# pierrenodet/spark-ensemble

Hardware: AMD Instinct MI355X
Metric: rows/sec (whole node) GBMClassifier 100 trees depth=8 at 1/2/4/8 MI355X (higher is better)
Workload: dtype fp32; 1 GPU; model=GBMClassifier(bernoulli, 265 trees, depth=8, bins=256), global_batch=10000000, rows_per_gpu=10000000, features=256, parallelism=dp1

## Files before the change

csrc/hist_plan.h:

```cpp
#pragma once

#include <algorithm>
#include <cmath>
#include <cstddef>
#include <cstdint>
#include <cstdlib>
#include <limits>
#include <stdexcept>
#include <vector>

struct HistPlan {
  int64_t chunk_rows = 0;
  int n_chunks = 0;
  int header_words = 0;
  std::vector<int> table;
  std::vector<int> multi_nodes;
};

inline HistPlan plan_hist_chunks(const int64_t* offs, int n_nodes,
                                 const int* col0 ,
                                 int64_t row_bound, int col_bound,
                                 size_t lds_bytes, int n_groups,
                                 int header_words) {
  int64_t total_rows = 0;
  for (int nd = 0; nd < n_nodes; ++nd) {
    const int64_t s = offs[nd], e = offs[nd + 1];
    if (s < 0 || e < s || e > row_bound ||
        e > std::numeric_limits<int>::max())
      throw std::invalid_argument("hist plan: node_offsets out of range");
    const int c0 = col0 ? col0[nd] : 0;
    if (c0 < 0 || c0 >= col_bound)
      throw std::invalid_argument("hist plan: node_col0 out of range");
    total_rows += e - s;
  }

  const int blocks_per_cu =
      std::max<int>(1, (int)(163840 / std::max<size_t>(1, lds_bytes)));
  const int64_t resident = (int64_t)256 * blocks_per_cu;
  static const double oversub_env = []() {
    const char* e = getenv("SEA_HIST_OVERSUB");
    return e ? atof(e) : 0.0;
  }();
  const double oversub =
      oversub_env > 0 ? oversub_env : (blocks_per_cu == 1 ? 1.0 : 1.5);
  const int64_t target_chunks = std::max<int64_t>(
      1, (int64_t)(resident * oversub) / std::max(1, n_groups));

  HistPlan p;
  p.chunk_rows = std::max<int64_t>(
      4096, (total_rows + target_chunks - 1) / target_chunks);
  p.chunk_rows = std::min<int64_t>(p.chunk_rows, 1 << 20);
  p.header_words = header_words;
  p.table.assign(header_words, 0);
  for (int nd = 0; nd < n_nodes; ++nd) {
    const int64_t s = offs[nd], e = offs[nd + 1];
    int slot = -1;
    if (e - s > p.chunk_rows) {
      slot = (int)p.multi_nodes.size();
      p.multi_nodes.push_back(nd);
    }
    int64_t c = s;
    do {
      const int rec[5] = {nd, (int)c,
                          (int)std::min<int64_t>(p.chunk_rows, e - c), slot,
                          col0 ? col0[nd] : 0};
      p.table.insert(p.table.end(), rec, rec + 5);
      c += p.chunk_rows;
    } while (c < e);
  }
  p.n_chunks = (int)((p.table.size() - header_words) / 5);
  return p;
}

inline double hist_fixed_scale(int64_t chunk_rows, double max_abs) {
  if (!(max_abs > 0.0) || !std::isfinite(max_abs)) max_abs = 1.0;
  const double s = (double)(1u << 30) / ((double)chunk_rows * max_abs);
  return std::min(s, (double)(1u << 30) / max_abs);
}
```

csrc/ops.hip:

```cpp

#include <ATen/hip/HIPContext.h>

#include <chrono>
#include <cstring>
#include <tuple>
#include <vector>

#include "common.h"
#include "hist_plan.h"

torch::Tensor h2d_async(const void* src, size_t bytes, UploadSlot slot,
                        const torch::Device& dev) {
  static thread_local torch::Tensor pin[2 * kUploadSlots];
  static thread_local hipEvent_t done[2 * kUploadSlots] = {};
  static thread_local unsigned char flip[kUploadSlots] = {};
  flip[slot] ^= 1;
  const int bi = slot * 2 + flip[slot];
  auto& b = pin[bi];
  if (done[bi]) (void)hipEventSynchronize(done[bi]);
  if (!b.defined() || (size_t)b.numel() < bytes) {
    size_t cap = 4096;
    while (cap < bytes) cap *= 2;
    b = torch::empty({(int64_t)cap},
                     torch::TensorOptions().dtype(torch::kByte)
// ... 98 lines not shown
      while (lo < hi) {
        const int mid = (lo + hi) >> 1;
        if (e[mid] >= v[j]) hi = mid; else lo = mid + 1;
      }
      b[j] = (uint8_t)lo;
    }
    if (full) {
      uint4 packed;
      unsigned* w = reinterpret_cast<unsigned*>(&packed);
#pragma unroll
      for (int q = 0; q < 4; ++q)
        w[q] = (unsigned)b[q * 4] | ((unsigned)b[q * 4 + 1] << 8) |
               ((unsigned)b[q * 4 + 2] << 16) | ((unsigned)b[q * 4 + 3] << 24);
      *reinterpret_cast<uint4*>(out + r * F + f0) = packed;
    } else {
      for (int j = 0; j < nf; ++j) out[r * F + f0 + j] = b[j];
    }
  }
}

void bin_features(torch::Tensor out, torch::Tensor x, torch::Tensor edges) {
  CHECK_GPU(out); CHECK_GPU(x); CHECK_GPU(edges);
  CHECK_CONTIG(out); CHECK_CONTIG(x); CHECK_CONTIG(edges);
  int64_t n = x.size(0);
  int F = (int)x.size(1);
  int nedges = (int)edges.size(1);
  TORCH_CHECK(nedges <= 1024, "bin_features: too many edges for LDS staging");
  auto stream = at::hip::getCurrentHIPStream();
  const int threads = 256;
  const int fgroups = (int)ceil_div(F, 16);
  int rblocks = (int)std::min<int64_t>(
      ceil_div(n, threads), std::max<int64_t>(1, 16384 / fgroups));
  const size_t lds = (size_t)16 * nedges * 4;
  hipLaunchKernelGGL(bin_features_kernel, dim3(rblocks, fgroups),
                     dim3(threads), lds, stream, out.data_ptr<uint8_t>(),
                     x.data_ptr<float>(), edges.data_ptr<float>(), n, F,
                     nedges);
}


__device__ inline void rotate_piece(unsigned (&w)[4], int lam) {
  const bool r1 = lam & 4, r2 = lam & 8;
  const unsigned a0 = r1 ? w[1] : w[0], a1 = r1 ? w[2] : w[1],
                 a2 = r1 ? w[3] : w[2], a3 = r1 ? w[0] : w[3];
  const unsigned b0 = r2 ? a2 : a0, b1 = r2 ? a3 : a1, b2 = r2 ? a0 : a2,
                 b3 = r2 ? a1 : a3;
  const unsigned t = lam & 3;
  w[0] = __builtin_amdgcn_alignbyte(b1, b0, t);
  w[1] = __builtin_amdgcn_alignbyte(b2, b1, t);
  w[2] = __builtin_amdgcn_alignbyte(b3, b2, t);
  w[3] = __builtin_amdgcn_alignbyte(b0, b3, t);
}

template <int DC, int NC, bool BM>
__global__ void hist_build_kernel(
    float* __restrict__ out,
    long long* __restrict__ stage,
    const uint8_t* __restrict__ bins,
    const float* __restrict__ gh,
    const int* __restrict__ row_idx,
    const int* __restrict__ chunks,
    int F, int B, int FG, int CH, int identity_rows) {
  constexpr int C = DC + NC;
  constexpr int CELLS = DC > NC ? DC : NC;
  extern __shared__ unsigned long long lds64[];
  const float* scales = reinterpret_cast<const float*>(chunks);
  const int* chk = chunks + 2 * C + blockIdx.x * 5;
  const int fg = blockIdx.y;
  const int f0 = fg * FG;
  const int nf = min(FG, F - f0);
  const int node = chk[0];
  const int start = chk[1];
  const int len = chk[2];
  const int slot = chk[3];
  const int col0 = chk[4];

  const int lds_cells = FG * B * CELLS;
  for (int i = threadIdx.x; i < lds_cells; i += blockDim.x) lds64[i] = 0ull;
  __syncthreads();

  constexpr int MAXNH = CELLS == 1 ? 4 : (CELLS == 2 ? 2 : 1);
  const int nh = FG >> 4;
  const int lam = threadIdx.x & 15;
  const int bshift = 31 - __clz(FG) + 3;
  const unsigned plane = (unsigned)B * FG * 8;
  unsigned foff[16];
#pragma unroll
  for (int p = 0; p < 16; ++p) foff[p] = ((p + lam) & 15) * 8;

  for (int i = threadIdx.x; i < len; i += blockDim.x) {
    const int r = identity_rows ? start + i : row_idx[start + i];
    const float* g = gh + (int64_t)r * CH + col0;
    unsigned long long addend[CELLS];
#pragma unroll
    for (int c = 0; c < CELLS; ++c) addend[c] = 0ull;
#pragma unroll
    for (int d = 0; d < DC; ++d) {
      const int iv = __float2int_rn(g[d] * scales[d]);
      addend[d] |= ((unsigned long long)(unsigned)iv) << 32;
    }
#pragma unroll
    for (int c = 0; c < NC; ++c) {
      const int iv = __float2int_rn(g[DC + c] * scales[DC + c]);
      addend[c] |= (unsigned)iv;
    }
    if constexpr (BM) {
      const uint8_t* br = bins + (int64_t)r * F + f0;
      uint4 bv[MAXNH];
#pragma unroll
      for (int hh = 0; hh < MAXNH; ++hh) {
        bv[hh] = make_uint4(0, 0, 0, 0);
        if (hh < nh) bv[hh] = *reinterpret_cast<const uint4*>(br + 16 * hh);
      }
      char* base = reinterpret_cast<char*>(lds64);
#pragma unroll
      for (int hh = 0; hh < MAXNH; ++hh) {
        if (hh >= nh) break;
        unsigned w[4] = {bv[hh].x, bv[hh].y, bv[hh].z, bv[hh].w};
        rotate_piece(w, lam);
#pragma unroll
        for (int p = 0; p < 16; ++p) {
          const unsigned b = (w[p >> 2] >> (8 * (p & 3))) & 0xff;
          char* cell = base + ((b << bshift) + foff[p]) + hh * 128;
#pragma unroll
          for (int c = 0; c < CELLS; ++c)
            atomicAdd(reinterpret_cast<unsigned long long*>(cell + c * plane),
                      addend[c]);
        }
      }
    } else {
      const uint8_t* br = bins + (int64_t)r * F + f0;
      for (int f = 0; f < nf; ++f) {
        const int b = br[f];
        unsigned long long* cell = lds64 + ((f * B) + b) * CELLS;
#pragma unroll
        for (int c = 0; c < CELLS; ++c) atomicAdd(cell + c, addend[c]);
      }
    }
  }
  __syncthreads();

  auto flush_cell = [&](int f, int b, const unsigned long long* cell,
                        int cstride) {
    if (slot < 0) {
      float* o = out + (((int64_t)node * F + f0 + f) * B + b) * C;
#pragma unroll
      for (int d = 0; d < DC; ++d)
        o[d] = (float)(int)(unsigned)(cell[d * cstride] >> 32) / scales[d];
#pragma unroll
      for (int c = 0; c < NC; ++c)
        o[DC + c] = (float)(int)(unsigned)(cell[c * cstride] & 0xFFFFFFFFull) /
                    scales[DC + c];
    } else {
      long long* o = stage + (((int64_t)slot * F + f0 + f) * B + b) * C;
#pragma unroll
      for (int d = 0; d < DC; ++d) {
        const int v = (int)(unsigned)(cell[d * cstride] >> 32);
        if (v) atomicAdd((unsigned long long*)(o + d),
                         (unsigned long long)(long long)v);
      }
#pragma unroll
      for (int c = 0; c < NC; ++c) {
        const int v = (int)(unsigned)(cell[c * cstride] & 0xFFFFFFFFull);
        if (v) atomicAdd((unsigned long long*)(o + DC + c),
                         (unsigned long long)(long long)v);
      }
    }
  };
  if constexpr (BM) {
    constexpr int TBL = 3;
    constexpr int TB = 1 << TBL, TF = 64 >> TBL;
    const int nbt = (B + TB - 1) >> TBL;
    const int n_tiles = (FG / TF) * nbt;
    for (int i = threadIdx.x; i < n_tiles * 64; i += blockDim.x) {
      const int t = i >> 6, l = i & 63;
      const int ft = t / nbt, bt = t - ft * nbt;
      const int f = ft * TF + (l >> TBL), b = bt * TB + (l & (TB - 1));
      if (b < B) flush_cell(f, b, lds64 + b * FG + f, B * FG);
    }
  } else {
    for (int i = threadIdx.x; i < nf * B; i += blockDim.x) {
      const int f = i / B, b = i - f * B;
      flush_cell(f, b, lds64 + ((f * B) + b) * CELLS, 1);
    }
  }
}

__global__ void hist_decode_kernel(float* __restrict__ out,
                                   const long long* __restrict__ stage,
                                   const int* __restrict__ nodes,
                                   const float* __restrict__ scales,
                                   int64_t FBC, int C) {
  const int64_t obase = (int64_t)nodes[blockIdx.y] * FBC;
  const int64_t sbase = (int64_t)blockIdx.y * FBC;
  for (int64_t i = blockIdx.x * (int64_t)blockDim.x + threadIdx.x; i < FBC;
       i += gridDim.x * (int64_t)blockDim.x) {
    const int c = (int)(i % C);
    out[obase + i] = (float)stage[sbase + i] / scales[c];
  }
}

void launch_hist_decode(float* out, const long long* stage, const int* nodes,
                        const float* scales, int n_multi, int64_t FBC, int C,
                        hipStream_t stream) {
  const int dblocks = (int)std::min<int64_t>(ceil_div(FBC, 256), 1024);
  hipLaunchKernelGGL(hist_decode_kernel, dim3(dblocks, n_multi), dim3(256), 0,
                     stream, out, stage, nodes, scales, FBC, C);
}

int64_t hist_build(torch::Tensor out, torch::Tensor bins, torch::Tensor gh,
                   torch::Tensor row_idx, torch::Tensor node_offsets,
                   int64_t num_bins, int64_t d_dims, torch::Tensor max_abs,
                   bool identity_rows, torch::Tensor node_col0,
                   int64_t c_per_node) {
  CHECK_GPU(out); CHECK_GPU(bins); CHECK_GPU(gh); CHECK_GPU(row_idx);
  CHECK_CONTIG(out); CHECK_CONTIG(bins); CHECK_CONTIG(gh); CHECK_CONTIG(row_idx);
  TORCH_CHECK(!node_offsets.is_cuda(), "node_offsets stays on host");
  TORCH_CHECK(!max_abs.is_cuda(), "max_abs stays on host");
  TORCH_CHECK(!node_col0.is_cuda(), "node_col0 stays on host");
  CHECK_CONTIG(node_offsets); CHECK_CONTIG(node_col0);
  const int F = (int)bins.size(1);
  const int B = (int)num_bins;
  const int CH = (int)gh.size(1);
  const int C = c_per_node > 0 ? (int)c_per_node : CH;
  const int n_nodes = (int)node_offsets.numel() - 1;
  const bool forest = node_col0.numel() > 0;
  TORCH_CHECK(!forest || node_col0.numel() == n_nodes,
              "node_col0 must have one entry per node");
  const int D = d_dims > 0 ? (int)d_dims : (C >= 3 ? C - 2 : C - 1);
  const int NN = C - D;
  TORCH_CHECK(C <= 8, "gh channels capped at 8 (grad dims + hess + count)");
  TORCH_CHECK(D >= 1 && NN >= 1 && NN <= 2,
              "hist_build: channels must be D grads + 1-2 nonneg, got C=", C,
              " D=", D);
  TORCH_CHECK(max_abs.numel() == C, "max_abs must have C entries");
  TORCH_CHECK(out.numel() == (int64_t)n_nodes * F * B * C,
              "out must be [n_nodes, F, B, C]");
  if (n_nodes == 0 || F == 0) return 0;
  const int CELLS = std::max(D, NN);

  static const int fg_env = []() {
    const char* e = getenv("SEA_HIST_FG");
    return e ? atoi(e) : 0;
  }();
  static const int lds_budget = []() {
    const char* e = getenv("SEA_HIST_LDS");
    return e ? atoi(e) : 163840;
  }();
  int FG = std::max<int>(1, std::min<int>(F, lds_budget / (B * CELLS * 8)));
  if (CELLS == 1 && FG >= 64 && (F % 64) == 0) FG = 64;
  else if (CELLS <= 2 && FG >= 32 && (F % 32) == 0) FG = 32;
  else if (FG >= 16) FG = 16;
  else if (FG >= 8) FG = 8;
  else if (FG >= 4) FG = 4;
  if (fg_env == 16 || fg_env == 32 || fg_env == 64)
    FG = std::min(FG, fg_env);
  const int threads =
      (FG >= 64 || (CELLS == 2 && FG >= 32)) ? 1024
      : ((FG >= 32 || (CELLS >= 3 && FG >= 16)) ? 512 : 256);
  const int n_groups = (int)ceil_div(F, FG);
  const size_t lds_bytes = (size_t)FG * B * CELLS * 8;

  HistPlan plan = plan_hist_chunks(
      node_offsets.data_ptr<int64_t>(), n_nodes,
      forest ? node_col0.data_ptr<int>() : nullptr,
      identity_rows ? bins.size(0) : row_idx.numel(), CH - C + 1, lds_bytes,
      n_groups, 2 * C);

  auto max_abs_f = max_abs.to(torch::kFloat32).contiguous();
  auto ma = max_abs_f.accessor<float, 1>();
  float* scales_f = reinterpret_cast<float*>(plan.table.data());
  for (int c = 0; c < C; ++c)
    scales_f[c] = (float)hist_fixed_scale(plan.chunk_rows, ma[c]);
  auto chunks = h2d_async(plan.table.data(), plan.table.size() * 4,
                          kSlotHistChunks, bins.device())
                    .view(torch::kInt32);

  const int n_multi = (int)plan.multi_nodes.size();
  torch::Tensor stage;
  long long* stage_ptr = nullptr;
  if (n_multi) {
    stage = torch::zeros({(int64_t)n_multi, (int64_t)F, (int64_t)B, (int64_t)C},
                         out.options().dtype(torch::kInt64));
    stage_ptr = reinterpret_cast<long long*>(stage.data_ptr<int64_t>());
  }

  auto stream = at::hip::getCurrentHIPStream();
  const bool bin_major =
      (FG == 16 || FG == 32 || FG == 64) && (F % FG) == 0;
  TORCH_CHECK(!bin_major || FG <= (CELLS == 1 ? 64 : (CELLS == 2 ? 32 : 16)),
              "hist_build: FG ", FG, " too wide for CELLS ", CELLS);
#define HB_LAUNCH_L(DD, NNN, BM)                                             \
  do {                                                                       \
    if (lds_bytes > 65536)                                                   \
      (void)hipFuncSetAttribute(                                             \
          reinterpret_cast<const void*>(&hist_build_kernel<DD, NNN, BM>),    \
          hipFuncAttributeMaxDynamicSharedMemorySize, (int)lds_bytes);       \
    hipLaunchKernelGGL((hist_build_kernel<DD, NNN, BM>),                     \
                       dim3(plan.n_chunks, n_groups), dim3(threads),         \
                       lds_bytes, stream, out.data_ptr<float>(), stage_ptr,  \
                       bins.data_ptr<uint8_t>(),                             \
                       gh.data_ptr<float>(), row_idx.data_ptr<int>(),        \
                       chunks.data_ptr<int>(), F, B, FG, CH,                 \
                       identity_rows ? 1 : 0);                               \
  } while (0)
#define HB_LAUNCH(DD, NNN)                                                   \
  do {                                                                       \
    if (bin_major) HB_LAUNCH_L(DD, NNN, true);                               \
    else HB_LAUNCH_L(DD, NNN, false);                                        \
  } while (0)
  const int key = D * 10 + NN;
  switch (key) {
    case 11: HB_LAUNCH(1, 1); break;
    case 12: HB_LAUNCH(1, 2); break;
    case 21: HB_LAUNCH(2, 1); break;
    case 22: HB_LAUNCH(2, 2); break;
    case 31: HB_LAUNCH(3, 1); break;
    case 32: HB_LAUNCH(3, 2); break;
    case 41: HB_LAUNCH(4, 1); break;
    case 42: HB_LAUNCH(4, 2); break;
    case 51: HB_LAUNCH(5, 1); break;
    case 52: HB_LAUNCH(5, 2); break;
    case 61: HB_LAUNCH(6, 1); break;
    case 62: HB_LAUNCH(6, 2); break;
    case 71: HB_LAUNCH(7, 1); break;
    default: TORCH_CHECK(false, "hist_build: unsupported D/NN ", D, "/", NN);
  }
#undef HB_LAUNCH
#undef HB_LAUNCH_L
  if (n_multi) {
    auto nodes = h2d_async(plan.multi_nodes.data(), (size_t)n_multi * 4,
                           kSlotHistNodes, bins.device());
    launch_hist_decode(out.data_ptr<float>(), stage_ptr,
                       (const int*)nodes.data_ptr(),
                       reinterpret_cast<const float*>(chunks.data_ptr<int>()),
                       n_multi, (int64_t)F * B * C, C, stream);
  }
  return n_multi;
}


__global__ void partition_kernel(
    int* __restrict__ new_rows,
    int* __restrict__ cursors,
    const uint8_t* __restrict__ bins,
    const uint8_t* __restrict__ bins_t,
    const int* __restrict__ row_idx,
    const int* __restrict__ chunks,
    const int* __restrict__ feat,
    const int* __restrict__ thr,
    int F, long long Nrows) {
  __shared__ int base_l, base_r, loc_l, loc_r;
  __shared__ int wl[8];
  extern __shared__ unsigned long long bits[];
  const int chunk = blockIdx.x;
  const int node = chunks[chunk * 3 + 0];
  const int start = chunks[chunk * 3 + 1];
  const int len = chunks[chunk * 3 + 2];
  const int f = feat[node];
  const int t = thr[node];
  const int lane = threadIdx.x & 63;
  const int wave = threadIdx.x >> 6;

  int my_l = 0;
  for (int i = threadIdx.x; i < ((len + 63) & ~63); i += blockDim.x) {
    const bool active = i < len;
    bool left = false;
    if (active) {
      const int r = row_idx[start + i];
      if (f < 0) {
        left = true;
      } else {
        const uint8_t bv = bins_t ? bins_t[(int64_t)f * Nrows + r]
                                  : bins[(int64_t)r * F + f];
        left = bv <= t;
      }
    }
    const unsigned long long m = __ballot(active && left);
    if (lane == 0) {
      bits[i >> 6] = m;
      my_l += (int)__popcll(m);
    }
  }
// ... 236 lines not shown
          const uint8_t bv = xt ? br[(int64_t)f * n] : br[f];
          go_left = bv <= (unsigned)(nd >> 32);
        } else {
          go_left = xr[f] <= __uint_as_float((unsigned)(nd >> 32));
        }
        node = toff + left + (go_left ? 0 : 1);
        nd = tlds[node];
        f = (short)(nd & 0xFFFFu);
      }
      if (D1) {
        acc1 += __uint_as_float((unsigned)(nd >> 32));
      } else {
        const float wt = w[first_tree + t];
        const float* lv = leaf + (int64_t)(node_base + node) * D;
        for (int d = 0; d < D; ++d) acc[d] += wt * lv[d];
      }
    }
    if (D1) {
      atomicAdd(out + r, acc1);
    } else {
      float* o = out + r * D;
      for (int d = 0; d < D; ++d)
        if (acc[d] != 0.0f) atomicAdd(o + d, acc[d]);
    }
  }
}


__device__ inline int seg_of(const long long* __restrict__ cum, int n_segs,
                             long long p) {
  int lo = 0, hi = n_segs;
  while (hi - lo > 1) {
    const int mid = (lo + hi) >> 1;
    if (cum[mid] <= p) lo = mid; else hi = mid;
  }
  return lo;
}

__global__ void gather_ranges_kernel(
    int* __restrict__ out,
    const int* __restrict__ src,
    const long long* __restrict__ seg,
    int n_segs, long long total) {
  const long long* cum = seg;
  const long long* starts = seg + n_segs + 1;
  const long long stride = (long long)gridDim.x * blockDim.x;
  for (long long p = (long long)blockIdx.x * blockDim.x + threadIdx.x;
       p < total; p += stride) {
    const int s = seg_of(cum, n_segs, p);
    out[p] = src[starts[s] + (p - cum[s])];
  }
}

__global__ void leaf_scatter_kernel(
    float* __restrict__ tp,
    const int* __restrict__ row_idx,
    const long long* __restrict__ seg,
    const int* __restrict__ tree,
    const float* __restrict__ val,
    int T, int n_segs, long long total) {
  const long long* cum = seg;
  const long long* starts = seg + n_segs + 1;
  const long long stride = (long long)gridDim.x * blockDim.x;
  for (long long p = (long long)blockIdx.x * blockDim.x + threadIdx.x;
       p < total; p += stride) {
    const int s = seg_of(cum, n_segs, p);
    const int r = row_idx[starts[s] + (p - cum[s])];
    tp[(long long)r * T + tree[s]] = val[s];
  }
}

void gather_ranges(torch::Tensor out, torch::Tensor src,
                   torch::Tensor starts, torch::Tensor lens) {
  CHECK_GPU(out); CHECK_GPU(src);
  const int n_segs = (int)starts.numel();
  const long long total = out.numel();
  if (n_segs == 0 || total == 0) return;
  auto st = starts.accessor<int64_t, 1>();
  auto ln = lens.accessor<int64_t, 1>();
  std::vector<long long> seg_v(2 * n_segs + 1);
  seg_v[0] = 0;
  for (int i = 0; i < n_segs; ++i) {
    seg_v[i + 1] = seg_v[i] + ln[i];
    seg_v[n_segs + 1 + i] = st[i];
  }
  TORCH_CHECK(seg_v[n_segs] == total, "gather_ranges: lens sum != out size");
  auto seg_b = h2d_async(seg_v.data(), seg_v.size() * 8, kSlotGatherSegs,
                         src.device());
  auto stream = at::hip::getCurrentHIPStream();
  const int blocks =
      (int)std::min<long long>(8192, ceil_div(total, (long long)1024));
  hipLaunchKernelGGL(gather_ranges_kernel, dim3(blocks), dim3(256), 0, stream,
                     out.data_ptr<int>(), src.data_ptr<int>(),
                     (const long long*)seg_b.data_ptr(), n_segs, total);
}

void leaf_scatter(torch::Tensor tp, torch::Tensor row_idx,
                  torch::Tensor starts, torch::Tensor lens,
                  torch::Tensor tree, torch::Tensor val) {
  CHECK_GPU(tp); CHECK_GPU(row_idx);
  const int n_segs = (int)starts.numel();
  if (n_segs == 0) return;
  const int T = (int)tp.size(1);
  auto st = starts.accessor<int64_t, 1>();
  auto ln = lens.accessor<int64_t, 1>();
  std::vector<long long> seg_v(2 * n_segs + 1);
  seg_v[0] = 0;
  for (int i = 0; i < n_segs; ++i) {
    seg_v[i + 1] = seg_v[i] + ln[i];
    seg_v[n_segs + 1 + i] = st[i];
  }
  const long long total = seg_v[n_segs];
  if (total == 0) return;
  auto seg_b = h2d_async(seg_v.data(), seg_v.size() * 8, kSlotLeafSegs,
                         tp.device());
  std::vector<int> tv(n_segs);
  std::vector<float> vv(n_segs);
  auto ta = tree.accessor<int64_t, 1>();
  auto va = val.accessor<float, 1>();
  for (int i = 0; i < n_segs; ++i) { tv[i] = (int)ta[i]; vv[i] = va[i]; }
  auto tree_b = h2d_async(tv.data(), tv.size() * 4, kSlotLeafTree, tp.device());
  std::vector<char> vb(n_segs * 4);
  std::memcpy(vb.data(), vv.data(), n_segs * 4);
  auto val_b = h2d_async(vb.data(), vb.size(), kSlotLeafVal, tp.device());
  auto stream = at::hip::getCurrentHIPStream();
  const int blocks =
      (int)std::min<long long>(8192, ceil_div(total, (long long)1024));
  hipLaunchKernelGGL(leaf_scatter_kernel, dim3(blocks), dim3(256), 0, stream,
                     tp.data_ptr<float>(), row_idx.data_ptr<int>(),
                     (const long long*)seg_b.data_ptr(),
                     (const int*)tree_b.data_ptr(),
                     (const float*)val_b.data_ptr(), T, n_segs, total);
}


__global__ void transpose_u8_kernel(uint8_t* __restrict__ out,
                                    const uint8_t* __restrict__ in,
                                    int64_t n, int F) {
  __shared__ uint8_t tile[64][68];
  const int64_t r0 = (int64_t)blockIdx.x * 64;
  const int f0 = blockIdx.y * 64;
  const int tid = threadIdx.x;
  const bool full = (r0 + 64 <= n) && (f0 + 64 <= F) && ((F & 3) == 0) &&
                    ((n & 3) == 0);
  if (full) {
    for (int i = tid; i < 1024; i += 256) {
      const int rr = i >> 4;
// ... 570 lines not shown
  if (C > 8) {
    CHECK_GPU(gain); CHECK_GPU(feat); CHECK_GPU(bin); CHECK_GPU(left_stats);
    split_argmax_wide(gain, feat, bin, left_stats, hist, D, lam,
                      min_child_weight, min_instances, min_info_gain);
    return;
  }
  auto best = torch::zeros({n}, hist.options().dtype(torch::kInt64));
  auto stream = at::hip::getCurrentHIPStream();
  const int fpb = 4;
#define SA_LAUNCH(CC)                                                         \
  do {                                                                        \
    hipLaunchKernelGGL(split_argmax_kernel<CC>,                               \
                       dim3(n, (F + fpb - 1) / fpb), dim3(64 * fpb), 0,       \
                       stream,                                                \
                       (unsigned long long*)best.data_ptr<int64_t>(),         \
                       hist.data_ptr<float>(), F, B, D, (float)lam,           \
                       (float)min_child_weight, (float)min_instances);        \
    hipLaunchKernelGGL(split_decode_kernel<CC>, dim3(n), dim3(64), 0, stream, \
                       gain.data_ptr<float>(), feat.data_ptr<int>(),          \
                       bin.data_ptr<int>(), left_stats.data_ptr<float>(),     \
                       (unsigned long long*)best.data_ptr<int64_t>(),         \
                       hist.data_ptr<float>(), F, B, (float)min_info_gain);   \
  } while (0)
  switch (C) {
    case 2: SA_LAUNCH(2); break;
    case 3: SA_LAUNCH(3); break;
    case 4: SA_LAUNCH(4); break;
    case 5: SA_LAUNCH(5); break;
    case 6: SA_LAUNCH(6); break;
    case 7: SA_LAUNCH(7); break;
    case 8: SA_LAUNCH(8); break;
  }
#undef SA_LAUNCH
}

std::tuple<int64_t, torch::Tensor, torch::Tensor> hist_plan_debug(
    torch::Tensor node_offsets, torch::Tensor node_col0, int64_t row_bound,
    int64_t col_bound, int64_t lds_bytes, int64_t n_groups) {
  auto offs = node_offsets.to(torch::kInt64).contiguous();
  auto col0 = node_col0.to(torch::kInt32).contiguous();
  const int n_nodes = (int)offs.numel() - 1;
  TORCH_CHECK(col0.numel() == 0 || col0.numel() == n_nodes,
              "node_col0 must be empty or have one entry per node");
  HistPlan plan = plan_hist_chunks(
      offs.data_ptr<int64_t>(), n_nodes,
      col0.numel() ? col0.data_ptr<int>() : nullptr, row_bound,
      (int)col_bound, (size_t)lds_bytes, (int)n_groups, 0);
  auto i32 = torch::TensorOptions().dtype(torch::kInt32);
  auto chunks = torch::tensor(plan.table, i32).view({plan.n_chunks, 5});
  auto multi = torch::tensor(plan.multi_nodes, i32);
  return {plan.chunk_rows, chunks, multi};
}

PYBIND11_MODULE(TORCH_EXTENSION_NAME, m) {
  m.def("_hist_plan", &hist_plan_debug,
        "host-side chunk plan of the histogram kernels (no device)");
  m.def("logreg_loss_grad", &logreg_loss_grad,
        "single-pass fused logistic loss+gradient");
  m.def("logreg_fused_supported", &logreg_fused_supported);
  m.def("split_argmax", &split_argmax,
        "fused best-split gain scan + argmax over node histograms");
  m.def("sample_weights", &sample_weights, "counter-based Poisson/Bernoulli row weights");
  m.def("bin_features", &bin_features, "quantile binning f32 -> u8");
  m.def("hist_build", &hist_build, "LDS-staged node histograms");
  m.def("hist_build_class", &hist_build_class,
        "label-indexed node histograms for K-class gini trees");
  m.def("partition_rows", &partition_rows, "block-aggregated node partition");
  m.def("tree_predict", &tree_predict, "single-tree batched predict");
  m.def("forest_predict", &forest_predict, "packed-forest weighted predict");
  m.def("forest_predict2", &forest_predict2,
        "LDS-staged tree-group-tiled forest predict");
  m.def("transpose_u8", &transpose_u8, "tiled u8 matrix transpose");
  m.def("gather_ranges", &gather_ranges,
        "one-pass concat of contiguous index ranges");
  m.def("leaf_scatter", &leaf_scatter,
        "scatter per-segment leaf values into the [N, T] train-pred matrix");
  m.def("grad_hess", &grad_hess, "fused per-row loss gradient/hessian");
  m.def("line_search_eval", &line_search_eval, "fused loss+grad line-search payload");
  m.def("newton_chain_1d", &newton_chain_1d,
        "device-chained safeguarded-Newton stage-weight search");
}
```

spark_ensemble_amd/models/tree_grower.py:

```python

from __future__ import annotations

from dataclasses import dataclass
from typing import Dict, List, Optional, Tuple

import torch

from ..ops import dispatch as ops
from ..parallel import Comm


@dataclass
class GrowParams:
    max_depth: int = 5
    max_bins: int = 32
    min_instances_per_node: int = 1
    min_info_gain: float = 0.0
    min_child_weight: float = 0.0
    lam: float = 1e-6


def ensure_binned(frame, x: torch.Tensor, max_bins: int):
    cached = frame.cache_get("bins", x, max_bins) if frame is not None else None
    if cached is not None:
# ... 612 lines not shown
        denom = (h + params.lam).unsqueeze(1)
        vals = torch.where(denom > 0, g / denom, torch.zeros_like(g))
        leaves_t[t_ids, nids] = vals
        if capture:
            starts = offs[idx_t]
            lens = offs[idx_t + 1] - starts
            nz = (lens > 0).nonzero(as_tuple=True)[0]
            if nz.numel():
                ops.leaf_scatter(tp_arena, ridx, starts[nz], lens[nz],
                                 t_ids[nz], vals[nz, 0])

    for depth in range(params.max_depth + 1):
        n_active = int(node_tree.numel())
        if n_active == 0:
            break
        if depth == params.max_depth:
            _finalize_and_capture(torch.arange(n_active), offsets, row_idx)
            break

        split_args = dict(
            lam=params.lam,
            min_child_weight=params.min_child_weight,
            min_instances=params.min_instances_per_node,
            min_info_gain=params.min_info_gain,
            d_dims=D,
        )
        lvl_mask = None
        if feature_masks is not None:
            lvl_mask = feature_masks.index_select(
                0, _to_dev_async(node_tree, device)
            )
        if hists is None:
            if class_mode:
                new_h = _class_hist(row_idx, offsets, node_tree,
                                    identity=(root_rows is None and T == 1))
            else:
                new_h = ops.hist_build_forest(
                    bins, gh, row_idx, offsets,
                    (node_tree * C).to(torch.int32), B, C, gh_max, d_dims=D,
                )
            hists, gain, feat, b, left_stats = _finish_level_split(
                new_h, None, None, None, None, None, n_active, (F, B, C),
                device, comm, split_args, split_mask=lvl_mask,
            )
        else:
            built_cpu = built_mask_t.nonzero(as_tuple=True)[0]
            nb_cpu = (~built_mask_t).nonzero(as_tuple=True)[0]
            bh = None
            if built_cpu.numel():
                starts = offsets[built_cpu]
                lens = offsets[built_cpu + 1] - starts
                b_off = torch.zeros(built_cpu.numel() + 1, dtype=torch.int64)
                b_off[1:] = torch.cumsum(lens, 0)
                build_rows = ops.gather_ranges(row_idx, starts, lens)
                if class_mode:
                    bh = _class_hist(build_rows, b_off, node_tree[built_cpu])
                else:
                    col0_b = (node_tree[built_cpu] * C).to(torch.int32)
                    bh = ops.hist_build_forest(
                        bins, gh, build_rows, b_off, col0_b, B, C, gh_max,
                        d_dims=D,
                    )
            hists, gain, feat, b, left_stats = _finish_level_split(
                bh, _to_dev_async(built_cpu, device), hists,
                _to_dev_async(nb_cpu, device),
                _to_dev_async(nb_cpu ^ 1, device),
                _to_dev_async(parent_of_t[nb_cpu], device), n_active,
                (F, B, C), device, comm, split_args, split_mask=lvl_mask,
            )
        pack_d = torch.cat([
            gain, feat.to(torch.float32), b.to(torch.float32),
            left_stats.reshape(-1),
        ])
        ev = None
        if bins.is_cuda:
            pack_h = torch.empty(pack_d.numel(), dtype=torch.float32,
                                 pin_memory=True)
            pack_h.copy_(pack_d, non_blocking=True)
            ev = torch.cuda.Event()
            ev.record()

        pr_async = None
        if bins.is_cuda:
            pr_async = ops.partition_rows_async(bins, row_idx, offsets, feat, b)

        if pending_writes is not None:
            pending_writes()
            pending_writes = None

        if ev is not None:
            ev.synchronize()
            pack = pack_h
        else:
            pack = pack_d
        gain_cpu = pack[:n_active]
        feat_cpu = pack[n_active:2 * n_active].to(torch.int32)
        b_cpu = pack[2 * n_active:3 * n_active].to(torch.int32)
        left_stats = pack[3 * n_active:].reshape(n_active, C)

        do_split = torch.isfinite(gain_cpu)
        ns_idx = (~do_split).nonzero(as_tuple=True)[0]
        _finalize_and_capture(ns_idx, offsets, row_idx)
        if not bool(do_split.any()):
            break

        s_idx = do_split.nonzero(as_tuple=True)[0]
        t_ids = node_tree[s_idx]
        nids = node_nid[s_idx]
        f_l = feat_cpu[s_idx].long()
        b_l = b_cpu[s_idx].long()
        counts = torch.bincount(t_ids, minlength=T)
        firsts = torch.cumsum(counts, 0) - counts
        rank = torch.arange(s_idx.numel(), dtype=torch.long) - firsts[t_ids]
        cid = cur_len[t_ids] + 2 * rank
# ... 80 lines not shown
```

spark_ensemble_amd/ops/dispatch.py:

```python

from __future__ import annotations

import os
from typing import Optional

import torch

from . import reference

_hip = None
_hip_error: Optional[str] = None


def _load_hip():
    global _hip, _hip_error
    if _hip is not None or _hip_error is not None:
        return _hip
    try:
        from . import hip_ext

        _hip = hip_ext.load()
    except Exception as e:
        _hip_error = f"{type(e).__name__}: {e}"
        _hip = None
# ... 43 lines not shown
            out = torch.empty(x.shape, dtype=torch.uint8, device=x.device)
            m.bin_features(out, x.contiguous(), edges.contiguous())
            return out
    return reference.bin_features(x, edges)


def hist_build(bins, gh, row_idx, node_offsets, num_bins, d_dims=-1, max_abs=None, identity_rows=False):
    if bins.is_cuda:
        m = _require_hip("hist_build")
        if m is not None:
            n_nodes = node_offsets.numel() - 1
            C = gh.shape[1]
            if max_abs is None:
                max_abs = gh.abs().amax(dim=0).cpu()
            if C > 8:
                D = d_dims if d_dims > 0 else C - 1
                tail = list(range(D, C))
                step = 8 - len(tail)
                assert 1 <= step <= 7, f"hist_build tail too wide: {len(tail)}"
                spans = []
                cols: list = []
                for s in range(0, D, step):
                    w = min(step, D - s)
                    spans.append((len(cols), w))
                    cols.extend(range(s, s + w))
                    cols.extend(tail)
                idx = torch.tensor(cols, device=gh.device)
                gh_wide = gh.index_select(1, idx).contiguous()
                ma_wide = max_abs[torch.tensor(cols)]
                parts = []
                for ci, (c0, w) in enumerate(spans):
                    cc = w + len(tail)
                    part = hist_build_forest(
                        bins, gh_wide, row_idx, node_offsets,
                        torch.full((n_nodes,), c0, dtype=torch.int32),
                        num_bins, cc, ma_wide[c0:c0 + cc], d_dims=w,
                    )
                    parts.append(part[..., :w])
                    if ci == len(spans) - 1:
                        parts.append(part[..., w:])
                return torch.cat(parts, dim=-1)
            return _hist_build_launch(
                m, bins, gh, row_idx, node_offsets, _EMPTY_I32, num_bins, C,
                max_abs, d_dims, identity_rows,
            )
    return reference.hist_build(bins, gh, row_idx, node_offsets, num_bins)


_EMPTY_I32 = torch.empty(0, dtype=torch.int32)
_EMPTY_U8 = torch.empty(0, dtype=torch.uint8)


def _hist_build_launch(m, bins, gh, row_idx, node_offsets, node_col0,
                       num_bins, c_per_node, max_abs, d_dims, identity_rows):
    out = torch.empty(
        node_offsets.numel() - 1, bins.shape[1], num_bins, c_per_node,
        dtype=torch.float32, device=bins.device,
    )
    m.hist_build(
        out, bins, gh.contiguous(), row_idx.to(torch.int32),
        node_offsets.to(torch.int64).cpu().contiguous(), int(num_bins),
        int(d_dims), max_abs.to(torch.float32), bool(identity_rows),
        node_col0, int(c_per_node),
    )
    return out


def hist_build_forest(bins, gh, row_idx, node_offsets, node_col0, num_bins,
                      c_per_node, max_abs, d_dims=1):
    if bins.is_cuda:
        m = _require_hip("hist_build")
        if m is not None:
            return _hist_build_launch(
                m, bins, gh, row_idx, node_offsets,
                node_col0.to(torch.int32).cpu().contiguous(), num_bins,
                c_per_node, max_abs, d_dims, False,
            )
    return reference.hist_build_forest(
        bins, gh, row_idx, node_offsets, node_col0, num_bins, c_per_node
    )


last_hist_build_class_info: dict = {}


def hist_build_class(bins, label, weight, row_idx, node_offsets, node_col0,
                     num_bins, num_classes, nn, w_max=None,
                     identity_rows=False, transposed=None):
    if bins.is_cuda:
        m = _require_hip("hist_build_class")
        if m is not None:
            n_nodes = node_offsets.numel() - 1
            F = bins.shape[1]
            C = int(num_classes) + int(nn)
            if w_max is None:
                w_max = float(weight.max()) if weight.numel() else 1.0
            if transposed is None:
                transposed = os.environ.get("SEA_CLASS_HIST_SRC") != "rowmajor"
            bt = _bins_transposed(bins) if transposed else _EMPTY_U8
            out = torch.empty(n_nodes, F, num_bins, C, dtype=torch.float32,
                              device=bins.device)
            n_multi = m.hist_build_class(
                out, bins, bt, label, weight.contiguous(),
                row_idx.to(torch.int32),
                node_offsets.to(torch.int64).cpu().contiguous(),
                node_col0.to(torch.int32).cpu().contiguous(),
                int(num_bins), int(num_classes), int(nn), float(w_max),
                bool(identity_rows),
            )
            last_hist_build_class_info["multi_chunk_nodes"] = int(n_multi)
            return out
    return reference.hist_build_class(
        bins, label, weight, row_idx, node_offsets, node_col0, num_bins,
        num_classes, nn,
    )


SPLIT_WIDE_MAX_C = 34


def split_search(hist, lam=1e-6, min_child_weight=0.0, min_instances=1.0, min_info_gain=0.0, d_dims=-1):
    if hist.is_cuda:
        c_chk = hist.shape[3]
        if c_chk > SPLIT_WIDE_MAX_C:
            return reference.split_search(
                hist, lam, min_child_weight, min_instances, min_info_gain,
                d_dims,
            )
        m = _require_hip("split_argmax")
        if m is not None:
# ... 44 lines not shown


def partition_rows_async(bins, row_idx, node_offsets, feat, thr):
    import time as _time

    _prof = os.environ.get("SEA_GROW_PROF") == "1"
    _t0 = _time.perf_counter() if _prof else 0.0
    m = _require_hip("partition_rows")
    n = node_offsets.numel() - 1
    offs_cpu = node_offsets.to(torch.int64).cpu()
    row_idx = row_idx.to(torch.int32)
    new_rows = torch.empty_like(row_idx)
    left_counts = torch.zeros(n, dtype=torch.int32, device=bins.device)
    f32 = feat.to(torch.int32).to(bins.device)
    t32 = thr.to(torch.int32).to(bins.device)
    if _prof:
        _t1 = _time.perf_counter()
    bt = _bins_transposed(bins)
    m.partition_rows(
        new_rows,
        left_counts,
        bins,
        bt if bt is not None else _EMPTY_U8,
        row_idx,
        offs_cpu,
        f32,
        t32,
    )
    lc_h = torch.empty(left_counts.numel(), dtype=torch.int32,
                       pin_memory=True)
    lc_h.copy_(left_counts, non_blocking=True)
    ev = torch.cuda.Event()
    ev.record()
    if _prof:
        _t2 = _time.perf_counter()
        print(f"[part prof] prep={(_t1-_t0)*1000:.2f} native={(_t2-_t1)*1000:.2f}")
    return new_rows, (lc_h, ev), offs_cpu


def gather_ranges(src, starts, lens):
    if src.is_cuda:
        m = _require_hip("gather_ranges")
        if m is not None:
            out = torch.empty(int(lens.sum()), dtype=torch.int32,
                              device=src.device)
            m.gather_ranges(out, src, starts.to(torch.int64),
                            lens.to(torch.int64))
            return out
    st, ln = starts.tolist(), lens.tolist()
    segs = [src[s:s + l] for s, l in zip(st, ln) if l > 0]
    if not segs:
        return torch.empty(0, dtype=src.dtype, device=src.device)
    return segs[0].clone() if len(segs) == 1 else torch.cat(segs)


def leaf_scatter(tp, row_idx, starts, lens, tree, val):
    if tp.is_cuda:
        m = _require_hip("leaf_scatter")
        if m is not None:
            m.leaf_scatter(tp, row_idx, starts.to(torch.int64),
                           lens.to(torch.int64), tree.to(torch.int64),
                           val.to(torch.float32))
            return
    st, ln = starts.tolist(), lens.tolist()
    tl, vl = tree.tolist(), val.tolist()
    for s, l, t, v in zip(st, ln, tl, vl):
        if l > 0:
            tp[row_idx[s:s + l].long(), int(t)] = float(v)


def partition_rows_finish(new_rows, left_counts, offs_cpu):
    n = offs_cpu.numel() - 1
    if isinstance(left_counts, tuple):
        lc_h, ev = left_counts
        ev.synchronize()
        lc = lc_h.to(torch.int64)
    else:
        lc = left_counts.cpu().to(torch.int64)
    sizes = torch.empty(2 * n, dtype=torch.int64)
    seg = offs_cpu[1:] - offs_cpu[:-1]
    sizes[0::2] = lc
    sizes[1::2] = seg - lc
    new_offs = torch.cat([torch.zeros(1, dtype=torch.int64), sizes.cumsum(0)])
    return new_rows, new_offs, lc


def tree_predict(x, feature, threshold, left_child, leaf_value, max_depth):
    if x.is_cuda:
        m = _require_hip("tree_predict")
        if m is not None:
            N = x.shape[0]
            D = leaf_value.shape[1]
            out = torch.empty(N, D, dtype=torch.float32, device=x.device)
            m.tree_predict(
                out,
                x.contiguous(),
                feature.to(torch.int32).to(x.device),
                threshold.to(torch.float32).to(x.device),
                left_child.to(torch.int32).to(x.device),
                leaf_value.to(torch.float32).to(x.device).contiguous(),
            )
            return out
    return reference.tree_predict(x, feature, threshold, left_child, leaf_value, max_depth)


def forest_predict(x, trees, weights=None, max_depth=64, cache=None):
# ... 221 lines not shown
```

Measured before the change: 1.119 billion rows/sec.

## Gather compact gh per build row and replace atomic staging with slab reduce

The forest histogram path now gathers each build row's gradient/hessian slice into a compact, position-indexed buffer alongside the row indices, so the histogram kernel reads gh contiguously instead of by scattered row index. For single-cell histograms of multi-chunk nodes, each block writes its whole LDS image to a private slab instead of doing global 64-bit atomics, and a separate reduce kernel sums the slabs. A vectorized float4 flush is also added for two-component single-chunk nodes. This adds an extra gather pass, up to 1 GiB of scratch memory and another kernel launch in exchange for fewer random reads and less atomic contention.

```diff
diff --git a/csrc/hist_plan.h b/csrc/hist_plan.h
--- a/csrc/hist_plan.h
+++ b/csrc/hist_plan.h
@@ -15,6 +15,8 @@
   int header_words = 0;
   std::vector<int> table;
   std::vector<int> multi_nodes;
+  std::vector<int> slot_first;
+  std::vector<int> slot_count;
 };
 
 inline HistPlan plan_hist_chunks(const int64_t* offs, int n_nodes,
@@ -58,6 +60,8 @@
     if (e - s > p.chunk_rows) {
       slot = (int)p.multi_nodes.size();
       p.multi_nodes.push_back(nd);
+      p.slot_first.push_back((int)((p.table.size() - header_words) / 5));
+      p.slot_count.push_back((int)((e - s + p.chunk_rows - 1) / p.chunk_rows));
     }
     int64_t c = s;
     do {
diff --git a/csrc/ops.hip b/csrc/ops.hip
--- a/csrc/ops.hip
+++ b/csrc/ops.hip
@@ -174,15 +174,19 @@
   w[3] = __builtin_amdgcn_alignbyte(b0, b3, t);
 }
 
+template <int DC, int NC>
+constexpr bool kHistSlabFlush = (DC > NC ? DC : NC) == 1;
+
 template <int DC, int NC, bool BM>
 __global__ void hist_build_kernel(
     float* __restrict__ out,
     long long* __restrict__ stage,
+    unsigned long long* __restrict__ partial,
     const uint8_t* __restrict__ bins,
     const float* __restrict__ gh,
     const int* __restrict__ row_idx,
     const int* __restrict__ chunks,
-    int F, int B, int FG, int CH, int identity_rows) {
+    int F, int B, int FG, int CH, int identity_rows, int gh_pos) {
   constexpr int C = DC + NC;
   constexpr int CELLS = DC > NC ? DC : NC;
   extern __shared__ unsigned long long lds64[];
@@ -212,7 +216,7 @@
 
   for (int i = threadIdx.x; i < len; i += blockDim.x) {
     const int r = identity_rows ? start + i : row_idx[start + i];
-    const float* g = gh + (int64_t)r * CH + col0;
+    const float* g = gh + (int64_t)(gh_pos ? start + i : r) * CH + col0;
     unsigned long long addend[CELLS];
 #pragma unroll
     for (int c = 0; c < CELLS; ++c) addend[c] = 0ull;
@@ -290,6 +294,51 @@
     }
   };
   if constexpr (BM) {
+    if constexpr (kHistSlabFlush<DC, NC>) {
+      if (slot >= 0 && partial) {
+        const int* srec = chunks + 2 * C + (int)gridDim.x * 5 + slot * 4;
+        const int64_t slab =
+            (int64_t)(srec[3] + (int)blockIdx.x - srec[1]) * gridDim.y + fg;
+        uint4* dst = reinterpret_cast<uint4*>(partial + slab * lds_cells);
+        const uint4* img = reinterpret_cast<const uint4*>(lds64);
+        for (int i = threadIdx.x; i < lds_cells / 2; i += blockDim.x)
+          dst[i] = img[i];
+        return;
+      }
+    }
+    constexpr int NB = C == 2 ? 2 : 1;
+    if (NB > 1 && slot < 0 && B % NB == 0 &&
+        (reinterpret_cast<uintptr_t>(out) & 15) == 0) {
+      const int nbt = (B + 8 * NB - 1) / (8 * NB);
+      const int n_tiles = (FG >> 3) * nbt;
+      for (int i = threadIdx.x; i < n_tiles * 64; i += blockDim.x) {
+        const int t = i >> 6, l = i & 63;
+        const int ft = t / nbt, bt = t - ft * nbt;
+        const int f = ft * 8 + (l >> 3), b = (bt * 8 + (l & 7)) * NB;
+        if (b >= B) continue;
+        float v[NB * C];
+#pragma unroll
+        for (int k = 0; k < NB; ++k) {
+          const unsigned long long* cell = lds64 + (b + k) * FG + f;
+#pragma unroll
+          for (int d = 0; d < DC; ++d)
+            v[k * C + d] =
+                (float)(int)(unsigned)(cell[d * B * FG] >> 32) / scales[d];
+#pragma unroll
+          for (int c = 0; c < NC; ++c)
+            v[k * C + DC + c] =
+                (float)(int)(unsigned)(cell[c * B * FG] & 0xFFFFFFFFull) /
+                scales[DC + c];
+        }
+        float4* o = reinterpret_cast<float4*>(
+            out + (((int64_t)node * F + f0 + f) * B + b) * C);
+#pragma unroll
+        for (int q = 0; q < NB * C / 4; ++q)
+          o[q] = make_float4(v[4 * q], v[4 * q + 1], v[4 * q + 2],
+                             v[4 * q + 3]);
+      }
+      return;
+    }
     constexpr int TBL = 3;
     constexpr int TB = 1 << TBL, TF = 64 >> TBL;
     const int nbt = (B + TB - 1) >> TBL;
@@ -330,11 +379,51 @@
                      stream, out, stage, nodes, scales, FBC, C);
 }
 
+__global__ void hist_reduce_kernel(
+    float* __restrict__ out,
+    const unsigned long long* __restrict__ partial,
+    const int* __restrict__ slots,
+    const float* __restrict__ scales,
+    int F, int B, int FG, int DC, int NC) {
+  const int* srec = slots + blockIdx.y * 4;
+  const int node = srec[0], count = srec[2];
+  const int C = DC + NC, CELLS = DC > NC ? DC : NC;
+  const int n_groups = F / FG;
+  const int nbt = (B + 7) >> 3;
+  const int group_tiles = (FG >> 3) * nbt;
+  const int i = blockIdx.x * blockDim.x + threadIdx.x;
+  const int t = i >> 6, l = i & 63;
+  const int g = t / group_tiles;
+  if (g >= n_groups) return;
+  const int tt = t - g * group_tiles;
+  const int ft = tt / nbt, bt = tt - ft * nbt;
+  const int f = ft * 8 + (l >> 3), b = bt * 8 + (l & 7);
+  if (b >= B) return;
+  const int64_t plane = (int64_t)B * FG;
+  const int64_t kstride = (int64_t)n_groups * plane * CELLS;
+  const unsigned long long* p =
+      partial + ((int64_t)srec[3] * n_groups + g) * plane * CELLS + b * FG + f;
+  float* o = out + (((int64_t)node * F + g * FG + f) * B + b) * C;
+  for (int c = 0; c < CELLS; ++c) {
+    long long hi = 0, lo = 0;
+#pragma unroll 4
+    for (int k = 0; k < count; ++k) {
+      const unsigned long long v = p[k * kstride + c * plane];
+      hi += (int)(unsigned)(v >> 32);
+      lo += (int)(unsigned)(v & 0xFFFFFFFFull);
+    }
+    if (c < DC) o[c] = (float)hi / scales[c];
+    if (c < NC) o[DC + c] = (float)lo / scales[DC + c];
+  }
+}
+
+constexpr int64_t kHistPartialMaxBytes = (int64_t)1 << 30;
+
 int64_t hist_build(torch::Tensor out, torch::Tensor bins, torch::Tensor gh,
                    torch::Tensor row_idx, torch::Tensor node_offsets,
                    int64_t num_bins, int64_t d_dims, torch::Tensor max_abs,
                    bool identity_rows, torch::Tensor node_col0,
-                   int64_t c_per_node) {
+                   int64_t c_per_node, bool gh_by_position) {
   CHECK_GPU(out); CHECK_GPU(bins); CHECK_GPU(gh); CHECK_GPU(row_idx);
   CHECK_CONTIG(out); CHECK_CONTIG(bins); CHECK_CONTIG(gh); CHECK_CONTIG(row_idx);
   TORCH_CHECK(!node_offsets.is_cuda(), "node_offsets stays on host");
@@ -358,6 +447,9 @@
   TORCH_CHECK(max_abs.numel() == C, "max_abs must have C entries");
   TORCH_CHECK(out.numel() == (int64_t)n_nodes * F * B * C,
               "out must be [n_nodes, F, B, C]");
+  TORCH_CHECK(!gh_by_position ||
+                  (!identity_rows && gh.size(0) == row_idx.numel()),
+              "gh_by_position: gh must have one row per row_idx entry");
   if (n_nodes == 0 || F == 0) return 0;
   const int CELLS = std::max(D, NN);
 
@@ -389,6 +481,24 @@
       identity_rows ? bins.size(0) : row_idx.numel(), CH - C + 1, lds_bytes,
       n_groups, 2 * C);
 
+  const bool bin_major =
+      (FG == 16 || FG == 32 || FG == 64) && (F % FG) == 0;
+  TORCH_CHECK(!bin_major || FG <= (CELLS == 1 ? 64 : (CELLS == 2 ? 32 : 16)),
+              "hist_build: FG ", FG, " too wide for CELLS ", CELLS);
+
+  const int n_multi = (int)plan.multi_nodes.size();
+  const size_t slots_at = plan.table.size();
+  int64_t n_slabs = 0;
+  for (int s = 0; s < n_multi; ++s) {
+    const int rec[4] = {plan.multi_nodes[s], plan.slot_first[s],
+                        plan.slot_count[s], (int)n_slabs};
+    plan.table.insert(plan.table.end(), rec, rec + 4);
+    n_slabs += plan.slot_count[s];
+  }
+  const int64_t partial_bytes = n_slabs * n_groups * (int64_t)lds_bytes;
+  const bool use_partial = bin_major && CELLS == 1  &&
+                           n_multi && partial_bytes <= kHistPartialMaxBytes;
+
   auto max_abs_f = max_abs.to(torch::kFloat32).contiguous();
   auto ma = max_abs_f.accessor<float, 1>();
   float* scales_f = reinterpret_cast<float*>(plan.table.data());
@@ -398,20 +508,21 @@
                           kSlotHistChunks, bins.device())
                     .view(torch::kInt32);
 
-  const int n_multi = (int)plan.multi_nodes.size();
-  torch::Tensor stage;
+  torch::Tensor stage, partial;
   long long* stage_ptr = nullptr;
-  if (n_multi) {
+  unsigned long long* partial_ptr = nullptr;
+  if (use_partial) {
+    partial = torch::empty({partial_bytes / 8},
+                           out.options().dtype(torch::kInt64));
+    partial_ptr =
+        reinterpret_cast<unsigned long long*>(partial.data_ptr<int64_t>());
+  } else if (n_multi) {
     stage = torch::zeros({(int64_t)n_multi, (int64_t)F, (int64_t)B, (int64_t)C},
                          out.options().dtype(torch::kInt64));
     stage_ptr = reinterpret_cast<long long*>(stage.data_ptr<int64_t>());
   }
 
   auto stream = at::hip::getCurrentHIPStream();
-  const bool bin_major =
-      (FG == 16 || FG == 32 || FG == 64) && (F % FG) == 0;
-  TORCH_CHECK(!bin_major || FG <= (CELLS == 1 ? 64 : (CELLS == 2 ? 32 : 16)),
-              "hist_build: FG ", FG, " too wide for CELLS ", CELLS);
 #define HB_LAUNCH_L(DD, NNN, BM)                                             \
   do {                                                                       \
     if (lds_bytes > 65536)                                                   \
@@ -421,10 +532,10 @@
     hipLaunchKernelGGL((hist_build_kernel<DD, NNN, BM>),                     \
                        dim3(plan.n_chunks, n_groups), dim3(threads),         \
                        lds_bytes, stream, out.data_ptr<float>(), stage_ptr,  \
-                       bins.data_ptr<uint8_t>(),                             \
+                       partial_ptr, bins.data_ptr<uint8_t>(),                \
                        gh.data_ptr<float>(), row_idx.data_ptr<int>(),        \
                        chunks.data_ptr<int>(), F, B, FG, CH,                 \
-                       identity_rows ? 1 : 0);                               \
+                       identity_rows ? 1 : 0, gh_by_position ? 1 : 0);       \
   } while (0)
 #define HB_LAUNCH(DD, NNN)                                                   \
   do {                                                                       \
@@ -450,7 +561,15 @@
   }
 #undef HB_LAUNCH
 #undef HB_LAUNCH_L
-  if (n_multi) {
+  if (use_partial) {
+    const int64_t lanes = (int64_t)n_groups * (FG >> 3) * ((B + 7) >> 3) * 64;
+    hipLaunchKernelGGL(hist_reduce_kernel,
+                       dim3((unsigned)ceil_div(lanes, 256), n_multi),
+                       dim3(256), 0, stream, out.data_ptr<float>(),
+                       partial_ptr, chunks.data_ptr<int>() + slots_at,
+                       reinterpret_cast<const float*>(chunks.data_ptr<int>()),
+                       F, B, FG, D, NN);
+  } else if (n_multi) {
     auto nodes = h2d_async(plan.multi_nodes.data(), (size_t)n_multi * 4,
                            kSlotHistNodes, bins.device());
     launch_hist_decode(out.data_ptr<float>(), stage_ptr,
@@ -793,6 +912,27 @@
   }
 }
 
+__global__ void gather_ranges_gh_kernel(
+    int* __restrict__ out,
+    float* __restrict__ gh_out,
+    const int* __restrict__ src,
+    const float* __restrict__ gh,
+    const long long* __restrict__ seg,
+    int n_segs, long long total, int C, int CH) {
+  const long long* cum = seg;
+  const long long* starts = seg + n_segs + 1;
+  const long long* col0 = starts + n_segs;
+  const long long stride = (long long)gridDim.x * blockDim.x;
+  for (long long p = (long long)blockIdx.x * blockDim.x + threadIdx.x;
+       p < total; p += stride) {
+    const int s = seg_of(cum, n_segs, p);
+    const int r = src[starts[s] + (p - cum[s])];
+    out[p] = r;
+    const float* g = gh + (long long)r * CH + col0[s];
+    for (int c = 0; c < C; ++c) gh_out[p * C + c] = g[c];
+  }
+}
+
 __global__ void leaf_scatter_kernel(
     float* __restrict__ tp,
     const int* __restrict__ row_idx,
@@ -834,6 +974,48 @@
   hipLaunchKernelGGL(gather_ranges_kernel, dim3(blocks), dim3(256), 0, stream,
                      out.data_ptr<int>(), src.data_ptr<int>(),
                      (const long long*)seg_b.data_ptr(), n_segs, total);
+}
+
+void gather_ranges_gh(torch::Tensor out, torch::Tensor gh_out,
+                      torch::Tensor src, torch::Tensor gh,
+                      torch::Tensor starts, torch::Tensor lens,
+                      torch::Tensor col0) {
+  CHECK_GPU(out); CHECK_GPU(gh_out); CHECK_GPU(src); CHECK_GPU(gh);
+  CHECK_CONTIG(out); CHECK_CONTIG(gh_out); CHECK_CONTIG(src); CHECK_CONTIG(gh);
+  TORCH_CHECK(gh.dim() == 2 && gh_out.dim() == 2 &&
+                  gh_out.size(0) == out.numel(),
+              "gather_ranges_gh: gh_out must be [out.numel(), C]");
+  const int n_segs = (int)starts.numel();
+  const long long total = out.numel();
+  const int C = (int)gh_out.size(1), CH = (int)gh.size(1);
+  TORCH_CHECK(lens.numel() == n_segs && col0.numel() == n_segs,
+              "gather_ranges_gh: one len and col0 per range");
+  if (n_segs == 0 || total == 0) return;
+  auto st = starts.accessor<int64_t, 1>();
+  auto ln = lens.accessor<int64_t, 1>();
+  auto c0 = col0.accessor<int64_t, 1>();
+  std::vector<long long> seg_v(3 * n_segs + 1);
+  seg_v[0] = 0;
+  for (int i = 0; i < n_segs; ++i) {
+    TORCH_CHECK(ln[i] >= 0 && st[i] >= 0 && st[i] + ln[i] <= src.numel(),
+                "gather_ranges_gh: range outside src");
+    TORCH_CHECK(c0[i] >= 0 && c0[i] + C <= CH,
+                "gather_ranges_gh: col0 outside gh");
+    seg_v[i + 1] = seg_v[i] + ln[i];
+    seg_v[n_segs + 1 + i] = st[i];
+    seg_v[2 * n_segs + 1 + i] = c0[i];
+  }
+  TORCH_CHECK(seg_v[n_segs] == total,
+              "gather_ranges_gh: lens sum != out size");
+  auto seg_b = h2d_async(seg_v.data(), seg_v.size() * 8, kSlotGatherSegs,
+                         src.device());
+  auto stream = at::hip::getCurrentHIPStream();
+  const int blocks =
+      (int)std::min<long long>(8192, ceil_div(total, (long long)1024));
+  hipLaunchKernelGGL(gather_ranges_gh_kernel, dim3(blocks), dim3(256), 0,
+                     stream, out.data_ptr<int>(), gh_out.data_ptr<float>(),
+                     src.data_ptr<int>(), gh.data_ptr<float>(),
+                     (const long long*)seg_b.data_ptr(), n_segs, total, C, CH);
 }
 
 void leaf_scatter(torch::Tensor tp, torch::Tensor row_idx,
@@ -1510,9 +1692,30 @@
   return {plan.chunk_rows, chunks, multi};
 }
 
+std::tuple<torch::Tensor, torch::Tensor> hist_plan_slots_debug(
+    torch::Tensor node_offsets, torch::Tensor node_col0, int64_t row_bound,
+    int64_t col_bound, int64_t lds_bytes, int64_t n_groups) {
+  auto offs = node_offsets.to(torch::kInt64).contiguous();
+  auto col0 = node_col0.to(torch::kInt32).contiguous();
+  const int n_nodes = (int)offs.numel() - 1;
+  TORCH_CHECK(col0.numel() == 0 || col0.numel() == n_nodes,
+              "node_col0 must be empty or have one entry per node");
+  HistPlan plan = plan_hist_chunks(
+      offs.data_ptr<int64_t>(), n_nodes,
+      col0.numel() ? col0.data_ptr<int>() : nullptr, row_bound,
+      (int)col_bound, (size_t)lds_bytes, (int)n_groups, 0);
+  auto i32 = torch::TensorOptions().dtype(torch::kInt32);
+  return {torch::tensor(plan.slot_first, i32),
+          torch::tensor(plan.slot_count, i32)};
+}
+
 PYBIND11_MODULE(TORCH_EXTENSION_NAME, m) {
   m.def("_hist_plan", &hist_plan_debug,
         "host-side chunk plan of the histogram kernels (no device)");
+  m.def("_hist_plan_slots", &hist_plan_slots_debug,
+        "first record and record count of each staging slot of _hist_plan");
+  m.def("gather_ranges_gh", &gather_ranges_gh,
+        "gather_ranges plus the compact gh rows of the gathered rows");
   m.def("logreg_loss_grad", &logreg_loss_grad,
         "single-pass fused logistic loss+gradient");
   m.def("logreg_fused_supported", &logreg_fused_supported);
@@ -1520,7 +1723,11 @@
         "fused best-split gain scan + argmax over node histograms");
   m.def("sample_weights", &sample_weights, "counter-based Poisson/Bernoulli row weights");
   m.def("bin_features", &bin_features, "quantile binning f32 -> u8");
-  m.def("hist_build", &hist_build, "LDS-staged node histograms");
+  m.def("hist_build", &hist_build, "LDS-staged node histograms",
+        py::arg("out"), py::arg("bins"), py::arg("gh"), py::arg("row_idx"),
+        py::arg("node_offsets"), py::arg("num_bins"), py::arg("d_dims"),
+        py::arg("max_abs"), py::arg("identity_rows"), py::arg("node_col0"),
+        py::arg("c_per_node"), py::arg("gh_by_position") = false);
   m.def("hist_build_class", &hist_build_class,
         "label-indexed node histograms for K-class gini trees");
   m.def("partition_rows", &partition_rows, "block-aggregated node partition");
diff --git a/spark_ensemble_amd/models/tree_grower.py b/spark_ensemble_amd/models/tree_grower.py
--- a/spark_ensemble_amd/models/tree_grower.py
+++ b/spark_ensemble_amd/models/tree_grower.py
@@ -688,14 +688,18 @@
                 lens = offsets[built_cpu + 1] - starts
                 b_off = torch.zeros(built_cpu.numel() + 1, dtype=torch.int64)
                 b_off[1:] = torch.cumsum(lens, 0)
-                build_rows = ops.gather_ranges(row_idx, starts, lens)
                 if class_mode:
+                    build_rows = ops.gather_ranges(row_idx, starts, lens)
                     bh = _class_hist(build_rows, b_off, node_tree[built_cpu])
                 else:
-                    col0_b = (node_tree[built_cpu] * C).to(torch.int32)
+                    build_rows, gh_b = ops.gather_ranges_gh(
+                        row_idx, gh, starts, lens, node_tree[built_cpu] * C,
+                        C,
+                    )
                     bh = ops.hist_build_forest(
-                        bins, gh, build_rows, b_off, col0_b, B, C, gh_max,
-                        d_dims=D,
+                        bins, gh_b, build_rows, b_off,
+                        torch.zeros(built_cpu.numel(), dtype=torch.int32),
+                        B, C, gh_max, d_dims=D, gh_by_position=True,
                     )
             hists, gain, feat, b, left_stats = _finish_level_split(
                 bh, _to_dev_async(built_cpu, device), hists,
diff --git a/spark_ensemble_amd/ops/dispatch.py b/spark_ensemble_amd/ops/dispatch.py
--- a/spark_ensemble_amd/ops/dispatch.py
+++ b/spark_ensemble_amd/ops/dispatch.py
@@ -119,7 +119,8 @@
 
 
 def _hist_build_launch(m, bins, gh, row_idx, node_offsets, node_col0,
-                       num_bins, c_per_node, max_abs, d_dims, identity_rows):
+                       num_bins, c_per_node, max_abs, d_dims, identity_rows,
+                       gh_by_position=False):
     out = torch.empty(
         node_offsets.numel() - 1, bins.shape[1], num_bins, c_per_node,
         dtype=torch.float32, device=bins.device,
@@ -128,21 +129,27 @@
         out, bins, gh.contiguous(), row_idx.to(torch.int32),
         node_offsets.to(torch.int64).cpu().contiguous(), int(num_bins),
         int(d_dims), max_abs.to(torch.float32), bool(identity_rows),
-        node_col0, int(c_per_node),
+        node_col0, int(c_per_node), bool(gh_by_position),
     )
     return out
 
 
 def hist_build_forest(bins, gh, row_idx, node_offsets, node_col0, num_bins,
-                      c_per_node, max_abs, d_dims=1):
+                      c_per_node, max_abs, d_dims=1, gh_by_position=False):
     if bins.is_cuda:
         m = _require_hip("hist_build")
         if m is not None:
             return _hist_build_launch(
                 m, bins, gh, row_idx, node_offsets,
                 node_col0.to(torch.int32).cpu().contiguous(), num_bins,
-                c_per_node, max_abs, d_dims, False,
-            )
+                c_per_node, max_abs, d_dims, False, gh_by_position,
+            )
+    if gh_by_position:
+        pos = torch.arange(row_idx.numel(), device=row_idx.device)
+        return reference.hist_build_forest(
+            bins.index_select(0, row_idx.long()), gh, pos, node_offsets,
+            node_col0, num_bins, c_per_node
+        )
     return reference.hist_build_forest(
         bins, gh, row_idx, node_offsets, node_col0, num_bins, c_per_node
     )
@@ -293,6 +300,30 @@
     if not segs:
         return torch.empty(0, dtype=src.dtype, device=src.device)
     return segs[0].clone() if len(segs) == 1 else torch.cat(segs)
+
+
+def gather_ranges_gh(src, gh, starts, lens, col0, c_per_node):
+    C = int(c_per_node)
+    if src.is_cuda:
+        m = _require_hip("gather_ranges_gh")
+        if m is not None:
+            total = int(lens.sum())
+            out = torch.empty(total, dtype=torch.int32, device=src.device)
+            gh_out = torch.empty(total, C, dtype=torch.float32,
+                                 device=src.device)
+            m.gather_ranges_gh(out, gh_out, src, gh.contiguous(),
+                               starts.to(torch.int64), lens.to(torch.int64),
+                               col0.to(torch.int64))
+            return out, gh_out
+    rows = gather_ranges(src, starts, lens)
+    segs = [
+        gh[src[s:s + l].long(), c0:c0 + C]
+        for s, l, c0 in zip(starts.tolist(), lens.tolist(), col0.tolist())
+        if l > 0
+    ]
+    if not segs:
+        return rows, gh.new_empty(0, C)
+    return rows, torch.cat(segs)
 
 
 def leaf_scatter(tp, row_idx, starts, lens, tree, val):
```

After: 1.244 billion rows/sec (median of 6 runs). 1.11x the previous value.
